# debbiemarkslab/EVcouplings

Hardware: AMD Instinct MI355X
Metric: plmc L-BFGS iterations/sec (PLM fit, synthetic MSA) (higher is better)
Workload: dtype f32 (forward: f16 hi/lo split couplings on the 2:4 sparse MFMA, f32 accumulation -- in the last iterations of a fit 39-bit fixed-point couplings as five int8 digit planes, exact; backward: 24-bit fixed-point residuals as three int8 digit planes on the int8 MFMA (32-bit / four there), exact int32 acc; 1 GPU; headline: synthetic MSA L=300 q=21 N=50000, theta=0.8, lambda_h=0.01, lambda_J=59.8; parallelism=single GPU

## Files before the change

evcouplings_amd/csrc/plm_kernels.hip:

```cpp
#include "../../include/plm_hip.h"
#include "plm_internal.h"
#include <math.h>
#include <stdlib.h>
#include <string.h>
#include <mutex>
#include <utility>

typedef _Float16 half8 __attribute__((ext_vector_type(8)));
typedef _Float16 half4 __attribute__((ext_vector_type(4)));
typedef _Float16 half16 __attribute__((ext_vector_type(16)));
typedef float f32x4 __attribute__((ext_vector_type(4)));
typedef int i32x4 __attribute__((ext_vector_type(4)));
typedef unsigned int u32;

#ifndef PLM_DMA_STAGGER_FWD
#define PLM_DMA_STAGGER_FWD 4
#endif
#ifndef PLM_DMA_STAGGER_BWD
#define PLM_DMA_STAGGER_BWD 0
#endif
typedef unsigned long long u64;
#ifndef PLM_ASYNC_A
#define PLM_ASYNC_A 1
#endif
// ... 890 lines not shown
    const double *cref = (const double *)((const float *)(A.Bt + (size_t)d.blk_per_shard * d.nksteps * TILE_G) +
                                          (size_t)d.blk_per_shard * 16 * Q) + ((size_t)b16l * 16 + r) * Q + a_lo;
    auto value = [&](int m, int a, int e) -> float { return (float)__builtin_fma((double)sum64[m][a][e], sc64, cref[a]); };
    if constexpr (MODE == FWD_STORE) {
        float4 *hj = (float4 *)A.out + ((size_t)tile * 8 + wave) * 2 * Q * 64 + lane;
#pragma unroll
        for (int a = 0; a < QG; a++) {
#pragma unroll
            for (int m = 0; m < 2; m++)
                store_hj(&hj[(size_t)(m * Q + a_lo + a) * 64], value(m, a, 0), value(m, a, 1), value(m, a, 2), value(m, a, 3));
        }
    } else {
        const int i = b16 * 16 + r;
#pragma unroll
        for (int m = 0; m < 2; m++) {
#pragma unroll
            for (int reg = 0; reg < 4; reg++) {
                const int s = s_wave + 16 * m + 4 * g + reg;
                if (i < d.L && s < d.N) {
                    float *o = A.out + ((size_t)s * d.L + i) * d.Qc + a_lo;
#pragma unroll
                    for (int a = 0; a < QG; a++)
                        if (a_lo + a < d.Qc) o[a] = value(m, a, reg);
                }
            }
        }
    }
}

template <auto KERNEL> static hipError_t plm_allow_lds(size_t lds) {
    static std::once_flag once[PLM_MAX_DEVICES];
    static hipError_t result[PLM_MAX_DEVICES];
    const int dev = plm_current_device();
    std::call_once(once[dev], [&] {
        result[dev] = lds > 65536 ? hipFuncSetAttribute((const void *)KERNEL, hipFuncAttributeMaxDynamicSharedMemorySize, (int)lds)
                                  : hipSuccess;
    });
    return result[dev];
}

#ifndef PLM_FWDW_INC
#define PLM_FWDW_INC "plm_fwd_asm.inc"
#endif
#include PLM_FWDW_INC
template <int IDX> __device__ __forceinline__ f32x4 fwdw_acc_read() {
    f32x4 v;
    asm volatile("v_accvgpr_read_b32 %0, a[%4]\n\tv_accvgpr_read_b32 %1, a[%5]\n\t"
                 "v_accvgpr_read_b32 %2, a[%6]\n\tv_accvgpr_read_b32 %3, a[%7]"
                 : "=v"(v[0]), "=v"(v[1]), "=v"(v[2]), "=v"(v[3])
                 : "n"(IDX), "n"(IDX + 1), "n"(IDX + 2), "n"(IDX + 3));
    return v;
}
template <int M, int A>
__device__ __forceinline__ void fwdw_store(float4 *hj, const float *chi, const float *clo, float sc32) {
    const f32x4 v = fwdw_acc_read<(M * PLM_FWDW_QG + A) * 4>();
    const float h = chi[A], l = clo[A];
    store_hj(&hj[(size_t)((M & 1) * 21 + A) * 64 + (size_t)(M >> 1) * 2 * 21 * 64],
             __builtin_fmaf(v[0], sc32, l) + h, __builtin_fmaf(v[1], sc32, l) + h,
             __builtin_fmaf(v[2], sc32, l) + h, __builtin_fmaf(v[3], sc32, l) + h);
}
template <int M, int... A>
__device__ __forceinline__ void fwdw_store_row(float4 *hj, const float *chi, const float *clo, float sc32, std::integer_sequence<int, A...>) {
    (fwdw_store<M, A>(hj, chi, clo, sc32), ...);
}
template <int... M>
__device__ __forceinline__ void fwdw_store_all(float4 *hj, const float *chi, const float *clo, float sc32, std::integer_sequence<int, M...>) {
    (fwdw_store_row<M>(hj, chi, clo, sc32, std::make_integer_sequence<int, PLM_FWDW_QG>{}), ...);
}

__global__ __launch_bounds__(256) void k_fwd_w(PlmDims d, FwdArgs A) {
    extern __shared__ __attribute__((aligned(16))) char smem[];
    constexpr int Q = 21, QG = PLM_FWDW_QG, NSG = Q / QG, NM = PLM_FWDW_NM, SLOT = PLM_FWDW_SLOT;
    constexpr int TILE_G = 2 * Q * 1024, NG = PLM_FWD_NG(Q), SPU = 2 * NG;
    static_assert(NG == 5 && 2 * 2 * QG * 1024 == SLOT, "plm_fwd_asm.inc is generated for 21 states in groups of 7");
    const int tid = threadIdx.x, lane = tid & 63;
    const int wv = __builtin_amdgcn_readfirstlane(tid >> 6);
    const int npair = (d.nstiles + 1) >> 1;
    const int nwork = npair * (d.b16_hi - d.b16_lo) * NSG, per_xcd = (nwork + 7) >> 3;
    const int wk = (int)(blockIdx.x & 7) * per_xcd + (int)(blockIdx.x >> 3);
    if ((int)(blockIdx.x >> 3) >= per_xcd || wk >= nwork) return;
    const int spair = wk % npair, sg = (wk / npair) % NSG, b16l = wk / (npair * NSG);
    const int a_lo = sg * QG;
    const int r = lane & 15, g = lane >> 4;
    const int stile = 2 * spair + (wv >> 1);
    const bool tile_ok = stile < d.nstiles;
    const int s_wave = tile_ok ? stile * PLM_SEQ_TILE + (wv & 1) * 128 : 0;
    const int nsteps = d.nu * SPU;
    const char *bt = A.Bt + (size_t)b16l * nsteps * 2 * TILE_G + (size_t)a_lo * 1024 + wv * 1024;
    const u32 arow = (u32)(s_wave + r) * (u32)d.Lp32 + 8 * g, rstride = 16 * (u32)d.Lp32;

    const u32 l16 = (u32)lane * 16;
    u32 vo[PLM_FWDW_NVMEM];
#pragma unroll
    for (int k = 0; k < PLM_FWDW_NVMEM; k++) {
        const int p = wv + 4 * k, run = p / QG, f = p - run * QG;
        vo[k] = l16 + (u32)((run >> 1) * TILE_G + (run & 1) * Q * 1024 + f * 1024) - (u32)wv * 1024;
    }
    const u32 lw = lds_addr(smem + lane * 16);
    const u32 lw_base = __builtin_amdgcn_readfirstlane(lw - l16);
    const u32 m0t0 = lw_base + wv * 1024;
    const u32 cnt = lw_base + 4 * SLOT;
    if (tid == 0) *(u32 *)(smem + 4 * SLOT) = 0;
    const u32 one = 1, sel = 0x0c0c0200u;
    u32 st, sp;
    asm volatile(PLM_FWDW_ZERO_ASM ::: PLM_FWDW_CLOBBERS);
    for (int i = 0; i < 3; i++) {
        const int stepc = min(i, nsteps - 1);
        asm volatile(PLM_FWDW_ISSUE_ASM
                     :
                     : [tsrc] "s"(bt + (size_t)stepc * 2 * TILE_G), [vo0] "v"(vo[0]), [vo1] "v"(vo[1]), [vo2] "v"(vo[2]),
                       [vo3] "v"(vo[3]), [vo4] "v"(vo[4]), [vo5] "v"(vo[5]), [vo6] "v"(vo[6]), [m0t] "s"(m0t0 + i * SLOT)
                     : "m0", "scc", "memory");
    }
    asm volatile(PLM_FWDW_LOADS_ASM : : [arow] "v"(arow), [rstride] "s"(rstride), [xsrc] "s"(A.msa_rm) : PLM_FWDW_CLOBBERS);
    asm volatile(PLM_FWDW_UPREP_ASM
                 :
                 : [arow] "v"(arow), [rstride] "s"(rstride), [xsrc] "s"(A.msa_rm + 32 * min(1, d.nu - 1)), [sel] "s"(sel)
                 : PLM_FWDW_CLOBBERS);
    vm_wait<0>();
    __syncthreads();
    asm volatile(PLM_FWDW_PRIME_ASM : : [kg] "s"(0), [lbn] "v"(lw) : PLM_FWDW_CLOBBERS);

    int sc = 0;
    u32 tgt = 0;
    const char *tsrc = bt + (size_t)min(3, nsteps - 1) * 2 * TILE_G;
    int step = 0;
#define FWDW_SLICE(WHICH, KG)                                                                                          \
    {                                                                                                                  \
        const int sn = (sc + 1) & 3, snn = (sc + 3) & 3;                                                               \
        asm volatile(WHICH                                                                                             \
                     : [st] "=&s"(st), [sp] "=&s"(sp)                                                                  \
                     : [lb] "v"(lw + sc * SLOT), [lbn] "v"(lw + sn * SLOT), [kg] "s"(KG), [tsrc] "s"(tsrc),          \
                       [vo0] "v"(vo[0]), [vo1] "v"(vo[1]), [vo2] "v"(vo[2]), [vo3] "v"(vo[3]), [vo4] "v"(vo[4]),       \
                       [vo5] "v"(vo[5]), [vo6] "v"(vo[6]), [m0t] "s"(m0t0 + snn * SLOT), [cnt] "v"(cnt),               \
                       [one] "v"(one), [tgt] "s"(tgt)                                                                  \
                     : PLM_FWDW_CLOBBERS);                                                                             \
        sc = sn;                                                                                                       \
        tgt += 4;                                                                                                      \
        tsrc += (step + 4 < nsteps) ? (size_t)2 * TILE_G : 0;               \
        ++step;                                                                                                        \
    }
    for (int u = 0; u < d.nu; ++u) {
#pragma unroll 1
        for (int k = 0; k < NG; ++k) {
            FWDW_SLICE(PLM_FWDW_EVEN_ASM, k)
            if (k == NG - 1)
                asm volatile(PLM_FWDW_UPREP_ASM
                             :
                             : [arow] "v"(arow), [rstride] "s"(rstride),
                               [xsrc] "s"(A.msa_rm + 32 * min(u + 2, d.nu - 1)), [sel] "s"(sel)
                             : PLM_FWDW_CLOBBERS);
            FWDW_SLICE(PLM_FWDW_ODD_ASM, k + 1 < NG ? k + 1 : 0)
        }
    }
#undef FWDW_SLICE
    asm volatile("s_waitcnt vmcnt(0) lgkmcnt(0)\n\ts_nop 15\n\ts_nop 15" ::: "memory");
    if (!tile_ok) return;
    const int je = *A.jexp;
    const double sc64 = ldexp(1.0, -je);
    const double *cref = (const double *)((const float *)(A.Bt + (size_t)d.blk_per_shard * d.nksteps * TILE_G) +
                                          (size_t)d.blk_per_shard * 16 * Q) + ((size_t)b16l * 16 + r) * Q + a_lo;
    float4 *hj = (float4 *)A.out + ((size_t)(b16l * d.nstiles + stile) * 8 + (wv & 1) * 4) * 2 * Q * 64 + (size_t)a_lo * 64 + lane;
    float chi[QG], clo[QG];
#pragma unroll
    for (int a = 0; a < QG; a++) {
        const double c = cref[a];
        chi[a] = (float)c;
        clo[a] = (float)(c - (double)chi[a]);
    }
    fwdw_store_all(hj, chi, clo, (float)sc64, std::make_integer_sequence<int, NM>{});
}

int plm_fwd_groups(int q, int exact) {
    if (!exact) return q == 32 ? 2 : 1;
    return q == 32 ? 8 : q == 21 ? 3 : q == 20 ? 4 : 1;
}
template <int Q, int MODE, int NSG, bool EXACT>
static hipError_t fwd_launch(const PlmDims &d, const FwdArgs &A, hipStream_t st) {
    const int nwork = d.nstiles * (d.b16_hi - d.b16_lo) * NSG;
    const dim3 grid(8 * ((nwork + 7) / 8)), block(512);
    const size_t lds = (size_t)2 * 2 * (Q / NSG) * 1024;
    if constexpr (EXACT) {
        hipError_t e = plm_allow_lds<k_fwd_x<Q, MODE, NSG>>(lds);
        if (e != hipSuccess) return e;
        hipLaunchKernelGGL((k_fwd_x<Q, MODE, NSG>), grid, block, lds, st, d, A);
    } else {
        hipError_t e = plm_allow_lds<k_fwd<Q, MODE, NSG>>(lds);
        if (e != hipSuccess) return e;
        hipLaunchKernelGGL((k_fwd<Q, MODE, NSG>), grid, block, lds, st, d, A);
    }
    return hipGetLastError();
}
static hipError_t fwdw_launch(const PlmDims &d, const FwdArgs &A, hipStream_t st) {
    const int nwork = ((d.nstiles + 1) / 2) * (d.b16_hi - d.b16_lo) * (21 / PLM_FWDW_QG);
    const size_t lds = (size_t)4 * PLM_FWDW_SLOT + 16;
    hipError_t e = plm_allow_lds<k_fwd_w>(lds);
    if (e != hipSuccess) return e;
    hipLaunchKernelGGL(k_fwd_w, dim3(8 * ((nwork + 7) / 8)), dim3(256), lds, st, d, A);
    return hipGetLastError();
}
static hipError_t launch_forward_mode(const PlmDims &d, const FwdArgs &A, int mode, int exact, hipStream_t st) {
    if (d.b16_hi <= d.b16_lo) return hipSuccess;
#define FWD_CASE(QQ, NP, NX)       \
    case QQ:                                                                                           \
        if (mode == FWD_ENERGY) return fwd_launch<QQ, FWD_ENERGY, NP, false>(d, A, st);                \
        if (mode == FWD_POTENTIALS && exact) return fwd_launch<QQ, FWD_POTENTIALS, NX, true>(d, A, st); \
        if (mode == FWD_POTENTIALS) return fwd_launch<QQ, FWD_POTENTIALS, NP, false>(d, A, st);        \
        if (exact) return fwd_launch<QQ, FWD_STORE, NX, true>(d, A, st);                               \
        if (QQ == 21 && d.fwd_w) return fwdw_launch(d, A, st);                                         \
        return fwd_launch<QQ, FWD_STORE, NP, false>(d, A, st);
    switch (d.Q) {
        FWD_CASE(32, 2, 8)
        FWD_CASE(21, 1, 3)
        FWD_CASE(20, 1, 4)
        FWD_CASE(5, 1, 1)
        FWD_CASE(4, 1, 1)
    default:
        return hipErrorInvalidValue;
    }
#undef FWD_CASE
}
hipError_t plm_launch_forward_energy(const PlmDims &d, const int8_t *msa_rm, const void *Bt, const float *x,
                                     const int32_t *jexp, int potentials, int exact, float *out, hipStream_t st) {
    const FwdArgs A{msa_rm, (const char *)Bt, x, jexp, out};
    return launch_forward_mode(d, A, potentials ? FWD_POTENTIALS : FWD_ENERGY, potentials ? exact : 0, st);
}
hipError_t plm_launch_forward_store(const PlmDims &d, const int8_t *msa_rm, const void *Bt, const int32_t *jexp,
                                    float *hj, int exact, hipStream_t st) {
    const FwdArgs A{msa_rm, (const char *)Bt, nullptr, jexp, hj};
    return launch_forward_mode(d, A, FWD_STORE, exact, st);
}
size_t plm_hj_bytes(const PlmDims &d) { return (size_t)d.nstiles * (d.b16_hi - d.b16_lo) * 8 * 2 * d.Q * 1024; }

#define PLM_HSTATS(Q) ((Q) + (Q) * ((Q) + 1) / 2)
__host__ __device__ constexpr int plm_qc_min(int Q) { return Q == 4 ? 2 : Q == 5 ? 5 : Q == 20 ? 6 : Q == 21 ? 21 : 22; }
#ifndef PLM_HESS_SAMPLE
#define PLM_HESS_SAMPLE 32
#endif
#ifndef PLM_NEWTON_CAP
#define PLM_NEWTON_CAP 3.0
#endif
__device__ __forceinline__ float sum_over_g(float v) {
    unsigned u = __float_as_uint(v);
    auto a = __builtin_amdgcn_permlane32_swap(u, u, false, false);
    v = __uint_as_float(a[0]) + __uint_as_float(a[1]);
    u = __float_as_uint(v);
    auto b = __builtin_amdgcn_permlane16_swap(u, u, false, false);
    return __uint_as_float(b[0]) + __uint_as_float(b[1]);
}
__device__ __forceinline__ float log_unbiased(float z) {
    const float l2 = __builtin_amdgcn_logf(z);
    return __builtin_fmaf(l2, -1.904654323148236e-9f, l2 * 0.693147182464599609375f);
}
__device__ __forceinline__ float sel_eq(int x, int a, float if_ne, float if_eq) {
    float out;
    asm("v_cmp_eq_u32 vcc, %1, %2\n\tv_cndmask_b32 %0, %3, %4, vcc" : "=v"(out) : "s"(a), "v"(x), "v"(if_ne), "v"(if_eq) : "vcc");
    return out;
}
__device__ __forceinline__ void sel_eq2(int x, int a, float ne0, float eq0, float ne1, float eq1, float &o0, float &o1) {
    asm("v_cmp_eq_u32 vcc, %2, %3\n\tv_cndmask_b32 %0, %4, %5, vcc\n\tv_cndmask_b32 %1, %6, %7, vcc"
        : "=&v"(o0), "=&v"(o1) : "s"(a), "v"(x), "v"(ne0), "v"(eq0), "v"(ne1), "v"(eq1) : "vcc");
}
__global__ void k_sum_partials(const double *__restrict__ p, int n, double *out);
struct HpassArgs {
    const float4 *hj;
    const int8_t *msa_rm;
    const float *w;
    const double *h;
    int hstride;
    char *Rt;
    double *fx_part;
    float *hpart;
    double *gpart;
    float rscale;
    double *dpart;
    const int *state;
    int cond;
    int sel;
};
__device__ __forceinline__ bool vp_runs(const int *state, int cond) {
    if (!state || cond == PLM_VP_ALWAYS) return true;
    const PlmVpState *S = (const PlmVpState *)state;
    if (cond == PLM_VP_FINAL) return S->final_skip == 0;
    if (S->done) return false;
    return cond == PLM_VP_PASS_RT ? S->want_rt != 0 : S->want_rt == 0;
}
#define PLM_HESS_PARTS(Q) (((Q) == 20 || (Q) == 21) ? 3 : 1)
template <int Q> __host__ __device__ constexpr int hess_entry0(int a) { return a * Q - a * (a - 1) / 2; }
template <int Q> __host__ __device__ constexpr int hess_row_begin(int part) {
    if (part <= 0) return 0;
    if (part >= PLM_HESS_PARTS(Q)) return Q;
    int a = 0;
    while (a < Q && hess_entry0<Q>(a) * PLM_HESS_PARTS(Q) < part * (Q * (Q + 1) / 2)) a++;
    return a;
}
template <int Q> __host__ __device__ constexpr int hess_part_entries() {
    int m = 0;
    for (int p = 0; p < PLM_HESS_PARTS(Q); p++) {
        const int n = hess_entry0<Q>(hess_row_begin<Q>(p + 1)) - hess_entry0<Q>(hess_row_begin<Q>(p));
        m = n > m ? n : m;
    }
    return m;
}
template <int Q, bool WRITE_RT, int STATS, bool XACT>
__global__ __launch_bounds__(512) void k_hpass(PlmDims d, HpassArgs A) {
    extern __shared__ __attribute__((aligned(16))) char smem[];
    constexpr int NH = (STATS == 2) ? Q * (Q + 1) / 2 : 0;
    constexpr int NSP = (STATS == 2) ? PLM_HESS_PARTS(Q) : 1;
    constexpr int NHP = (STATS == 2) ? hess_part_entries<Q>() : 0;
    if (!vp_runs(A.state, A.cond)) return;
    if (A.state) A.h += (size_t)((const PlmVpState *)A.state)->cur * A.hstride;
    const int tid = threadIdx.x, lane = tid & 63;
    const int wave = __builtin_amdgcn_readfirstlane(tid >> 6);
    const int ns1 = (d.nstiles + PLM_HESS_SAMPLE - 1) / PLM_HESS_SAMPLE;
    const int sel = A.sel;
    const int part = (int)blockIdx.x % NSP, bid = (int)blockIdx.x / NSP;
    int row_lo = 0, row_hi = Q;
    if constexpr (NSP > 1) {
        row_lo = part == 0 ? 0 : (part == 1 ? hess_row_begin<Q>(1) : hess_row_begin<Q>(2));
        row_hi = part == 0 ? hess_row_begin<Q>(1) : (part == 1 ? hess_row_begin<Q>(2) : Q);
    }
    const int ent_lo = row_lo * Q - row_lo * (row_lo - 1) / 2, ent_hi = row_hi * Q - row_hi * (row_hi - 1) / 2;
    const int nst = sel == 0 ? d.nstiles : (sel == 1 ? ns1 : d.nstiles - ns1);
    const int kt = bid % nst, b16l = bid / nst;
    if (A.state && A.cond == PLM_VP_PASS && b16l < PLM_VP_MAXBLK && ((const PlmVpState *)A.state)->quiet[b16l]) return;
    const int stile = sel == 0 ? kt : (sel == 1 ? kt * PLM_HESS_SAMPLE : kt + kt / (PLM_HESS_SAMPLE - 1) + 1);
    constexpr int HW = Q > 21 ? 2 : 8;
    constexpr bool sampled = STATS == 2, DIAG = STATS == 3 || (STATS == 2 && Q > 21);
    const int blk = b16l * d.nstiles + stile;
    const int b16 = d.b16_lo + b16l;
    const int r = lane & 15, g = lane >> 4;
    const int s_wave = stile * PLM_SEQ_TILE + wave * 32;
    const int gap = d.gap_mode;
    const int i = b16 * 16 + r;
    const bool site_ok = i < d.L;
    float hv[XACT ? 1 : Q], hl[XACT ? 1 : Q];
    double hd[XACT ? Q : 1];
    auto load_fields = [&](bool opaque) {
        u32 hoff = (u32)(site_ok ? i - d.h_site0 : 0) * Q;
        if (opaque) asm volatile("" : "+v"(hoff));
#pragma unroll
        for (int a = 0; a < Q; a++) {
            const double h64 = site_ok ? A.h[hoff + a] : 0.0;
            if constexpr (XACT) {
                hd[a] = h64;
            } else {
                hv[a] = (float)h64;
                hl[a] = (float)(h64 - (double)hv[a]);
            }
        }
    };
    constexpr bool LDSF = !WRITE_RT && !XACT && (STATS != 2 || Q > 21);
    constexpr size_t STAT_BYTES = (size_t)16 * (8 * Q * sizeof(double) * (DIAG ? 2 : 1) + HW * NHP * sizeof(float));
    float2 *lf = (float2 *)(smem + STAT_BYTES);
    constexpr bool FAST = !WRITE_RT && !XACT && (STATS == 1 || STATS == 3);
    if constexpr (LDSF) {
        for (int k = tid; k < 16 * Q; k += 512) {
            const int ii = b16 * 16 + k / Q;
            const double h64 = ii < d.L ? A.h[(size_t)(ii - d.h_site0) * Q + k % Q] : 0.0;
            const float hi = (float)h64;
            lf[k] = make_float2(hi, (float)(h64 - (double)hi));
        }
        __syncthreads();
    } else if constexpr (!WRITE_RT) load_fields(false);
    float fxl = 0.f;
    double *lg = (double *)smem + ((size_t)wave * 16 + r) * Q;
    double *ld = lg + (size_t)8 * 16 * Q;
    float *lh0 = (float *)((double *)smem + (size_t)8 * 16 * Q * (DIAG ? 2 : 1));
    float *ls = lh0 + ((size_t)wave * 16 + r) * NHP;
    if (STATS) {
        for (int k = lane; k < 16 * Q; k += 64) ((double *)smem)[(size_t)wave * 16 * Q + k] = 0.0;
        if constexpr (sampled)
            if (wave < HW)
                for (int k = lane; k < 16 * NHP; k += 64) lh0[(size_t)wave * 16 * NHP + k] = 0.f;
        if constexpr (DIAG)
            for (int k = lane; k < 16 * Q; k += 64) ((double *)smem)[(size_t)(8 + wave) * 16 * Q + k] = 0.0;
    }
    const char *hj_u = (const char *)(A.hj + ((size_t)blk * 8 + wave) * 2 * Q * 64);
    const u32 lane16 = (u32)lane * 16;
    int m_end = 2;
    asm volatile("" : "+s"(m_end));
#pragma nounroll
    for (int m = 0; m < m_end; m++) {
        if constexpr (WRITE_RT) load_fields(true);
        f32x4 acc[Q];
#pragma unroll
        for (int a = 0; a < Q; a++) {
            const float4 v = *(const float4 *)(hj_u + (size_t)(m * Q + a) * 1024 + lane16);
            acc[a] = (f32x4){v.x, v.y, v.z, v.w};
        }
        float wk[4];
        float izk[4];
        int xk[4];
#pragma unroll
        for (int reg = 0; reg < 4; reg++) {
            const int s = s_wave + 16 * m + 4 * g + reg;
            const int xi = A.msa_rm[(size_t)s * d.Lp32 + i];
            const bool skip = gap && xi == 0;
            const float ws = (skip || !site_ok) ? 0.f : A.w[s];
            float mx = -INFINITY, Z = 0.f, hx = 0.f, zo = 0.f;
            if constexpr (!XACT) {
                u32 foff = (u32)r * Q;
                if constexpr (LDSF) asm volatile("" : "+v"(foff));
#pragma unroll
                for (int a = 0; a < Q; a++) {
                    float fh, fl;
                    if constexpr (LDSF) {
                        const float2 f = lf[foff + a];
                        fh = f.x;
                        fl = f.y;
                    } else {
                        fh = hv[a];
                        fl = hl[a];
                    }
                    const float H = ((gap && a == 0) || (a >= plm_qc_min(Q) && a >= d.Qc)) ? -INFINITY : (acc[a][reg] + fl) + fh;
                    acc[a][reg] = H;
                    mx = fmaxf(mx, H);
                }
                if constexpr (FAST) {
                    const float mxl = -mx * 1.44269502f;
#pragma unroll
                    for (int a = 0; a < Q; a++) {
                        const float ev = __builtin_amdgcn_exp2f(__builtin_fmaf(acc[a][reg], 1.44269502f, mxl));
                        const float evo = sel_eq(xi, a, ev, 0.f);
                        acc[a][reg] = evo;
                        Z += ev;
                        zo += evo;
                    }
                } else {
#pragma unroll
                    for (int a = 0; a < Q; a++) {
                        const float H = acc[a][reg] - mx;
                        const float ev = __expf(H);
                        float evo;
                        sel_eq2(xi, a, hx, H, ev, 0.f, hx, evo);
                        acc[a][reg] = ev;
                        Z += ev;
                        zo += evo;
                    }
                }
            } else {
#pragma unroll
                for (int a = 0; a < Q; a++) {
                    const float H = ((gap && a == 0) || a >= d.Qc) ? -INFINITY : acc[a][reg] + (float)hd[a];
                    mx = fmaxf(mx, H);
                }
                const double mxd = (double)mx;
#pragma unroll
                for (int a = 0; a < Q; a++) {
                    const double xs = ((double)acc[a][reg] + hd[a]) - mxd;
                    const double y = xs * 1.4426950408889634;
                    const float yh = (float)y, yl = (float)(y - (double)yh);
                    const float rr = __builtin_amdgcn_exp2f(yh);
                    const float ev = ((gap && a == 0) || a >= d.Qc) ? 0.f : __builtin_fmaf(rr, yl * 0.693147182464599609375f, rr);
                    float evo;
                    sel_eq2(xi, a, hx, (float)xs, ev, 0.f, hx, evo);
                    acc[a][reg] = ev;
                    Z += ev;
                    zo += evo;
                }
            }
            const float invZ = 1.f / Z;
            if (WRITE_RT && ws > 0.f) fxl -= ws * (hx - log_unbiased(Z));
            const float mpo = -(zo * invZ);
            if constexpr (FAST) {
                if (ws != 0.f) {
                    unsafeAtomicAdd(&lg[xi], (double)(ws * mpo));
                    if constexpr (STATS == 3) {
                        const float px = 1.f + mpo;
                        unsafeAtomicAdd(&ld[xi], (double)(ws * px * px));
                    }
                }
                wk[reg] = ws * invZ;
                izk[reg] = invZ;
                xk[reg] = xi;
            } else {
#pragma unroll
            for (int a = 0; a < Q; a++) acc[a][reg] = sel_eq(xi, a, acc[a][reg] * invZ, mpo);
            wk[reg] = ws;
            xk[reg] = xi;
            }
            asm volatile("" : "+v"(xk[reg]));
            if constexpr (XACT) __builtin_amdgcn_sched_barrier(0);
        }
        if constexpr (STATS != 0) {
            int idx = 0;
#pragma unroll
            for (int a = 0; a < Q; a++) {
                float t[4], ga = 0.f;
#pragma unroll
                for (int k = 0; k < 4; k++) {
                    t[k] = wk[k] * acc[a][k];
                    ga += t[k];
                }
#ifndef PLM_EXP_NOGRAD
                if (NSP == 1 || part == 0) unsafeAtomicAdd(&lg[a], (double)ga);
#else
                fxl += ga;
#endif
                if constexpr (DIAG) {
                    float da = 0.f;
                    if constexpr (FAST) {
#pragma unroll
                        for (int k = 0; k < 4; k++) da = fmaf(t[k] * acc[a][k], izk[k], da);
                    } else {
#pragma unroll
                    for (int k = 0; k < 4; k++) {
                        const bool obs = xk[k] == a;
                        da = fmaf(t[k] + (obs ? wk[k] : 0.f), acc[a][k] + (obs ? 1.f : 0.f), da);
                    }
                    }
#ifndef PLM_EXP_NOGRAD
                    unsafeAtomicAdd(&ld[a], (double)da);
#else
                    fxl += da;
#endif
                }
#ifndef PLM_EXP_NOHESS
                if (STATS == 2 && wave < HW && a >= row_lo && a < row_hi) {
                    idx = a * Q - a * (a - 1) / 2 - ent_lo;
#pragma unroll
                    for (int k = 0; k < 4; k++) t[k] += (xk[k] == a) ? wk[k] : 0.f;
#pragma unroll
                    for (int b = a; b < Q; b++) {
                        float v = 0.f;
#pragma unroll
                        for (int k = 0; k < 4; k++) v = fmaf(t[k], acc[b][k] + ((xk[k] == b) ? 1.f : 0.f), v);
#ifndef PLM_EXP_NOSWAP
                        v = sum_over_g(v);
#endif
#ifndef PLM_EXP_NOLDS
                        if (g == 0) __builtin_amdgcn_ds_faddf(LDS_FPTR(&ls[idx]), v, 0, 0, false);
#else
                        fxl += v;
#endif
                        ++idx;
                    }
                }
#endif
            }
        }
        if constexpr (WRITE_RT) {
            __builtin_amdgcn_sched_barrier(0);
            const int s64 = stile * 4 + (wave >> 1);
            const int Gq = 2 * (wave & 1) + m;
            char *rt_u = A.Rt + rt_slot(d, 0, s64, b16l * Q, 0);
            const size_t rt_plane = (size_t)d.nst128 * d.nnfl * 2048;
            const u32 slot16 = (u32)(Gq * 16 + r) * 16;
#pragma unroll
            for (int reg = 0; reg < 4; reg++) {
                wk[reg] *= A.rscale;
                asm volatile("" : "+v"(xk[reg]));
            }
            const bool four = d.nplanes == 4;
            auto planes_of_state = [&](int a, u32 (&pl)[PLM_BWD_MAXPLANES]) {
                u32 x[4];
#pragma unroll
                for (int reg = 0; reg < 4; reg++)
                    x[reg] = digits_of(wk[reg] * acc[a][reg], four);
                planes_of4(x[0], x[1], x[2], x[3], pl);
            };
#pragma unroll
            for (int q4 = 0; q4 + 4 <= Q; q4 += 4) {
                u32 pl[4][PLM_BWD_MAXPLANES];
#pragma unroll
                for (int k = 0; k < 4; k++) planes_of_state(q4 + k, pl[k]);
                const u32 off = (u32)(q4 + g) * 2048 + slot16;
#pragma unroll
                for (int p = 0; p < PLM_BWD_MAXPLANES; p++) {
                    if (p >= d.nplanes) break;
                    auto s02 = __builtin_amdgcn_permlane32_swap(pl[0][p], pl[2][p], false, false);
                    auto s13 = __builtin_amdgcn_permlane32_swap(pl[1][p], pl[3][p], false, false);
                    auto t0 = __builtin_amdgcn_permlane16_swap(s02[0], s13[0], false, false);
                    auto t1 = __builtin_amdgcn_permlane16_swap(s02[1], s13[1], false, false);
                    *(uint4 *)(rt_u + p * rt_plane + off) = make_uint4(t0[0], t0[1], t1[0], t1[1]);
                }
                __builtin_amdgcn_sched_barrier(0);
            }
#pragma unroll
            for (int a = Q - Q % 4; a < Q; a++) {
                u32 pl[PLM_BWD_MAXPLANES];
                planes_of_state(a, pl);
#pragma unroll
                for (int p = 0; p < PLM_BWD_MAXPLANES; p++)
                    if (p < d.nplanes) *(u32 *)(rt_u + p * rt_plane + (u32)a * 2048 + slot16 + 4 * g) = pl[p];
            }
        }
    }
    __syncthreads();
    if constexpr (STATS != 0) {
        if (NSP == 1 || part == 0) {
            double *gout = A.gpart + (size_t)blk * 16 * Q;
            for (int k = tid; k < 16 * Q; k += 512) {
                double v = 0;
#pragma unroll
                for (int wv = 0; wv < 8; wv++) v += ((const double *)smem)[(size_t)wv * 16 * Q + k];
                gout[k] = v;
            }
        }
        if constexpr (DIAG) {
            double *dout = A.dpart + (size_t)blk * 16 * Q;
            for (int k = tid; k < 16 * Q; k += 512) {
                double v = 0;
#pragma unroll
                for (int wv = 0; wv < 8; wv++) v += ((const double *)smem)[(size_t)(8 + wv) * 16 * Q + k];
                dout[k] = v;
            }
        }
        if constexpr (sampled) {
            float *out = A.hpart + (size_t)blk * 16 * NH;
            const int ne = ent_hi - ent_lo;
            for (int k = tid; k < 16 * ne; k += 512) {
                const int site = k / ne, e = k - site * ne;
                float v = 0.f;
#pragma unroll
                for (int wv = 0; wv < HW; wv++) v += lh0[((size_t)wv * 16 + site) * NHP + e];
                out[site * NH + ent_lo + e] = v;
            }
        }
    }
    if constexpr (WRITE_RT) {
        __syncthreads();
        const double tot = block_reduce_sum((double)fxl, (double *)smem);
        if (tid == 0) A.fx_part[blk] = tot;
    }
}
hipError_t plm_launch_hpass(const PlmDims &d, const float *hj, const int8_t *msa_rm, const float *w,
                            const double *h64, int write_rt, int stats, int exact, void *Rt, double *fx_part, float *hpart,
                            double *gpart, double *dpart, const int *state, int cond, hipStream_t st) {
    if (d.b16_hi <= d.b16_lo) return hipSuccess;
    const int nb = d.b16_hi - d.b16_lo, ns1 = (d.nstiles + PLM_HESS_SAMPLE - 1) / PLM_HESS_SAMPLE;
    const dim3 block(512);
    HpassArgs A{(const float4 *)hj, msa_rm, w, h64, (int)plm_h64_stride(d), (char *)Rt, fx_part,
                hpart, gpart, d.rscale, dpart, state, cond, 0};
#define HP_LAUNCH(QQ, WW, SS)                                                                          \
    {                                                                                                  \
        const dim3 grid((A.sel == 0 ? d.nstiles : (A.sel == 1 ? ns1 * ((SS) == 2 ? PLM_HESS_PARTS(QQ) : 1) : d.nstiles - ns1)) * nb); \
        const size_t lds = (size_t)16 * (8 * (QQ) * sizeof(double) * (((SS) == 3 || ((SS) == 2 && (QQ) > 21)) ? 2 : 1) + \
                                         ((SS) == 2 ? ((QQ) > 21 ? 2 : 8) * hess_part_entries<QQ>() : 0) * sizeof(float)) + \
                           (size_t)16 * (QQ) * sizeof(float2);           \
        {                                                                                              \
            hipError_t e = exact ? plm_allow_lds<k_hpass<QQ, WW, SS, true>>(lds) : plm_allow_lds<k_hpass<QQ, WW, SS, false>>(lds); \
            if (e != hipSuccess) return e;                                                             \
        }                                                                                              \
        if (exact) hipLaunchKernelGGL((k_hpass<QQ, WW, SS, true>), grid, block, lds, st, d, A);        \
        else hipLaunchKernelGGL((k_hpass<QQ, WW, SS, false>), grid, block, lds, st, d, A);             \
    }
#define HP_CASE(QQ)                                                                                    \
    case QQ:                                                                                           \
        if (write_rt && stats == 2) return hipErrorInvalidValue;    \
        else if (write_rt && stats == 0) HP_LAUNCH(QQ, true, 0)                                        \
        else if (write_rt) HP_LAUNCH(QQ, true, 1)                                                      \
        else if (stats == 2) {                                                                         \
            if (!dpart) return hipErrorInvalidValue;                                                   \
                         \
            A.sel = 1;                                                                                 \
            HP_LAUNCH(QQ, false, 2)                                                                    \
            A.sel = 2;                                                                                 \
            if (d.nstiles > ns1) HP_LAUNCH(QQ, false, 3)                                               \
        } else HP_LAUNCH(QQ, false, 1)                                                                 \
        break;
    switch (d.Q) {
        HP_CASE(32)
        HP_CASE(21)
        HP_CASE(20)
        HP_CASE(5)
        HP_CASE(4)
    default:
        return hipErrorInvalidValue;
    }
#undef HP_CASE
#undef HP_LAUNCH
    return hipGetLastError();
}
size_t plm_hpart_bytes(const PlmDims &d) {
    return (size_t)d.nstiles * (d.b16_hi - d.b16_lo) * 16 * (d.Q * (d.Q + 1) / 2) * sizeof(float);
}
size_t plm_h64_stride(const PlmDims &d) {
    const size_t nsites = (size_t)std::max(std::max(1, (d.b16_hi - d.b16_lo) * 16), std::min(d.L, d.own_hi * 16) - d.h_site0);
    return nsites * d.Q;
}
size_t plm_gpart_bytes(const PlmDims &d) { return (size_t)d.nstiles * (d.b16_hi - d.b16_lo) * 16 * d.Q * sizeof(double); }

template <int Q>
__global__ __launch_bounds__(256) void k_site_counts(PlmDims d, const int8_t *__restrict__ msa_cm, const float *__restrict__ w,
                                                    double *__restrict__ cnt) {
    __shared__ double red[4];
    const int il = blockIdx.x, i = d.h_site0 + il;
    double acc[Q];
#pragma unroll
    for (int a = 0; a < Q; a++) acc[a] = 0.0;
    if (i < d.L)
        for (int s = threadIdx.x; s < d.N; s += 256) {
            const int x = msa_cm[(size_t)i * d.Np + s];
            const double ws = (d.gap_mode && x == 0) ? 0.0 : (double)w[s];
#pragma unroll
            for (int a = 0; a < Q; a++) acc[a] += (x == a) ? ws : 0.0;
        }
#pragma unroll
    for (int a = 0; a < Q; a++) {
        const double t = block_reduce_sum(acc[a], red);
        if (threadIdx.x == 0) cnt[(size_t)il * Q + a] = t;
        __syncthreads();
    }
}
hipError_t plm_launch_site_counts(const PlmDims &d, const int8_t *msa_cm, const float *w, double *cnt, hipStream_t st) {
    const int nsites = (d.b16_hi - d.b16_lo) * 16;
    if (nsites <= 0) return hipSuccess;
    switch (d.Q) {
    case 32: hipLaunchKernelGGL(k_site_counts<32>, dim3(nsites), dim3(256), 0, st, d, msa_cm, w, cnt); break;
    case 21: hipLaunchKernelGGL(k_site_counts<21>, dim3(nsites), dim3(256), 0, st, d, msa_cm, w, cnt); break;
    case 20: hipLaunchKernelGGL(k_site_counts<20>, dim3(nsites), dim3(256), 0, st, d, msa_cm, w, cnt); break;
    case 5: hipLaunchKernelGGL(k_site_counts<5>, dim3(nsites), dim3(256), 0, st, d, msa_cm, w, cnt); break;
    case 4: hipLaunchKernelGGL(k_site_counts<4>, dim3(nsites), dim3(256), 0, st, d, msa_cm, w, cnt); break;
    default: return hipErrorInvalidValue;
    }
    return hipGetLastError();
}

template <int Q>
__global__ __launch_bounds__(64) void k_hsolve(PlmDims d, const float *__restrict__ hpart,
                                              const double *__restrict__ gpart, int full,
                                              float *__restrict__ x, double *__restrict__ h64,
                                              double lambda_h, int update,
                                              double *__restrict__ hinv, double *__restrict__ g2_site,
                                              double tol_site2, const int *__restrict__ state, int chain, int hstride,
                                              const double *__restrict__ cnt, const double *__restrict__ dpart) {
    constexpr int NVF = PLM_HSTATS(Q);
    const PlmVpState *S = (const PlmVpState *)state;
    int cur = 0;
    if (S) {
        if (chain && S->done) return;
        if (full == 2) full = S->want_rt ? 0 : 1;
        cur = S->cur;
    } else if (full == 2) full = 1;
    __shared__ double st[NVF];
    __shared__ double Hm[Q][2 * Q + 1];
    __shared__ double Hi[Q][Q + 1];
    __shared__ double gr[Q], Dv[Q], mv[Q], Md[Q];
    const int il = blockIdx.x, t = threadIdx.x;
    const int i = d.h_site0 + il;
    if (i >= min(d.L, d.own_hi * 16)) {
        if (t == 0) g2_site[il] = 0.0;
        return;
    }
    const double *hc = h64 + (size_t)cur * hstride + (size_t)il * Q;
    double *hn = h64 + (size_t)((S && chain) ? (cur ^ 1) : cur) * hstride + (size_t)il * Q;
    const int b16l = il >> 4, r = il & 15;
    const bool quiet = S && chain && b16l < PLM_VP_MAXBLK && S->quiet[b16l];
    if (quiet) {
        if (update && t < Q) hn[t] = hc[t];
        if (!S->want_rt) return;
        update = 0;
        full = 0;
    }
    constexpr int NH = Q * (Q + 1) / 2;
    {
        double part[Q];
#pragma unroll
        for (int k = 0; k < Q; k++) part[k] = 0;
        for (int tt = t; tt < d.nstiles; tt += 128) {
            const bool two = tt + 64 < d.nstiles;
            const double *src0 = gpart + (((size_t)b16l * d.nstiles + tt) * 16 + r) * Q;
            const double *src1 = gpart + (((size_t)b16l * d.nstiles + (two ? tt + 64 : tt)) * 16 + r) * Q;
            double v0[Q], v1[Q];
#pragma unroll
            for (int k = 0; k < Q; k++) { v0[k] = src0[k]; v1[k] = src1[k]; }
#pragma unroll
            for (int k = 0; k < Q; k++) { part[k] += v0[k]; if (two) part[k] += v1[k]; }
        }
#pragma unroll
        for (int k = 0; k < Q; k++) {
            double v = part[k];
            for (int o = 32; o > 0; o >>= 1) v += __shfl_xor(v, o, 64);
            if (t == 0) st[k] = v;
        }
    }
    if (full) {
        const int nsamp = (d.nstiles + PLM_HESS_SAMPLE - 1) / PLM_HESS_SAMPLE;
        for (int k = t; k < NH; k += 64) {
            double v = 0;
            for (int j0 = 0; j0 < nsamp; j0 += 8) {
                float u[8];
#pragma unroll
                for (int j = 0; j < 8; j++) {
                    const int tt = min(j0 + j, nsamp - 1) * PLM_HESS_SAMPLE;
                    u[j] = hpart[(((size_t)b16l * d.nstiles + tt) * 16 + r) * NH + k];
                }
#pragma unroll
                for (int j = 0; j < 8; j++)
                    if (j0 + j < nsamp) v += (double)u[j];
            }
            st[Q + k] = v * ((double)d.nstiles / nsamp) * (Q > 21 ? 4.0 : 1.0);
        }
        if (dpart) {
            double part[Q];
#pragma unroll
            for (int k = 0; k < Q; k++) part[k] = 0;
            for (int tt0 = t; tt0 < d.nstiles; tt0 += 128) {
                const bool two = tt0 + 64 < d.nstiles;
                double v[2][Q];
#pragma unroll
                for (int h = 0; h < 2; h++) {
                    const int tt = (h && two) ? tt0 + 64 : tt0;
                    const size_t blk = ((size_t)b16l * d.nstiles + tt) * 16 + r;
                    if (Q <= 21 && (tt % PLM_HESS_SAMPLE) == 0) {
#pragma unroll
                        for (int k = 0; k < Q; k++) v[h][k] = (double)hpart[blk * NH + (k * Q - k * (k - 1) / 2)];
                    } else {
#pragma unroll
                        for (int k = 0; k < Q; k++) v[h][k] = dpart[blk * Q + k];
                    }
                }
#pragma unroll
                for (int k = 0; k < Q; k++) { part[k] += v[0][k]; if (two) part[k] += v[1][k]; }
            }
#pragma unroll
            for (int k = 0; k < Q; k++) {
                double v = part[k];
                for (int o = 32; o > 0; o >>= 1) v += __shfl_xor(v, o, 64);
                if (t == 0) Md[k] = v;
            }
        }
    }
    __syncthreads();
    const int a0 = d.gap_mode;
    if (t < Q) gr[t] = (t < a0) ? 0.0 : st[t] + 2.0 * lambda_h * hc[t];
    __syncthreads();
    double *inv = hinv + (size_t)il * Q * Q;
    if (full) {
        for (int k = t; k < Q * Q; k += 64) {
            const int a = k / Q, b = k % Q, lo = min(a, b), hi = max(a, b);
            Hm[a][b] = -st[Q + lo * Q - lo * (lo - 1) / 2 + (hi - lo)];
            Hm[a][Q + b] = (a == b) ? 1.0 : 0.0;
        }
        __syncthreads();
        const bool xdiag = cnt && dpart;
        if (t < Q) {
            mv[t] = cnt ? fmax(0.0, st[t] + cnt[(size_t)il * Q + t]) : 0.0;
            if (xdiag) {
                mv[t] = fmax(0.0, mv[t] - Md[t]);
                Hm[t][t] = 0.0;
            }
            Dv[t] = 1.0;
        }
        __syncthreads();
        if (cnt) {
            for (int sweep = 0; sweep < 3; sweep++) {
                double nd = 0.0;
                if (t < Q) {
                    double rs = 0;
                    for (int b = 0; b < Q; b++) rs -= Hm[t][b] * Dv[b];
                    rs *= Dv[t];
                    nd = rs > 0.0 ? Dv[t] * sqrt(mv[t] / rs) : 0.0;
                }
                __syncthreads();
                if (t < Q) Dv[t] = nd;
                __syncthreads();
            }
            for (int k = t; k < Q * Q; k += 64) Hm[k / Q][k % Q] *= Dv[k / Q] * Dv[k % Q];
            __syncthreads();
        }
        if (t < Q) {
            double rowsum = 0;
            for (int b = 0; b < Q; b++) rowsum -= Hm[t][b];
            Hm[t][2 * Q] = rowsum;
        }
        __syncthreads();
        if (t < Q) Hm[t][t] += Hm[t][2 * Q] + 2.0 * lambda_h + 1e-12 * (1.0 + Hm[t][2 * Q]);
        __syncthreads();
        {
            double col[Q];
            const int tc = min(t, 2 * Q - 1);
#pragma unroll
            for (int a = 0; a < Q; a++) col[a] = Hm[a][tc];
#pragma unroll
            for (int p = 0; p < Q; p++) {
                const double piv = 1.0 / lane_bcast(col[p], p);
                col[p] *= piv;
#pragma unroll
                for (int a = 0; a < Q; a++) {
                    if (a == p) continue;
                    const double f = lane_bcast(col[a], p);
                    col[a] -= f * col[p];
                }
            }
            if (t >= Q && t < 2 * Q) {
#pragma unroll
                for (int a = 0; a < Q; a++) Hm[a][t] = col[a];
            }
            __syncthreads();
        }
    }
    double g2 = 0;
    for (int a = 0; a < Q; a++) g2 += gr[a] * gr[a];
    if (t == 0) g2_site[il] = g2;
    const bool move = update && g2 > tol_site2;
    if (!move && !full) {
        if (S && chain && update && t < Q) hn[t] = hc[t];
        return;
    }
    for (int k = t; k < Q * Q; k += 64) Hi[k / Q][k % Q] = full ? Hm[k / Q][Q + k % Q] : inv[k];
    __syncthreads();
    const bool dirty = full != 0;
    if (dirty) for (int k = t; k < Q * Q; k += 64) inv[k] = Hi[k / Q][k % Q];
    if (!move) {
        if (S && chain && update && t < Q) hn[t] = hc[t];
        return;
    }
    double dh = 0;
    if (t < Q) {
        for (int b = 0; b < Q; b++) dh += Hi[t][b] * gr[b];
        if (t < a0) dh = 0;
    }
    double mxs = fabs(dh);
    for (int o = 32; o > 0; o >>= 1) mxs = fmax(mxs, __shfl_xor(mxs, o, 64));
    const double cap = (mxs > PLM_NEWTON_CAP) ? PLM_NEWTON_CAP / mxs : 1.0;
    if (t < Q) {
        const bool bad = mxs != mxs;
        const double hnew = bad ? hc[t] : hc[t] - cap * dh;
        hn[t] = hnew;
        if (!(S && chain)) x[(size_t)il * Q + t] = (float)hnew;
    }
}
__global__ __launch_bounds__(256) void k_fields_to_x(const double *__restrict__ h64, const int *__restrict__ state, int hstride,
                                                    float *__restrict__ x, int n) {
    const int k = blockIdx.x * 256 + threadIdx.x;
    const int cur = state ? ((const PlmVpState *)state)->cur : 0;
    if (k < n) x[k] = (float)h64[(size_t)cur * hstride + k];
}
hipError_t plm_launch_fields_to_x(const PlmDims &d, const double *h64, const int *state, float *x, hipStream_t st) {
    const int n = (std::min(d.L, d.own_hi * 16) - d.h_site0) * d.Q;
    if (n <= 0) return hipSuccess;
    hipLaunchKernelGGL(k_fields_to_x, dim3((n + 255) / 256), dim3(256), 0, st, h64, state, (int)plm_h64_stride(d), x, n);
    return hipGetLastError();
}
__global__ __launch_bounds__(256) void k_h64_init(const float *__restrict__ x, double *__restrict__ h64, int n) {
    const int k = blockIdx.x * 256 + threadIdx.x;
    if (k < n) h64[k] = (double)x[k];
}
hipError_t plm_launch_h64_init(const PlmDims &d, const float *x, double *h64, hipStream_t st) {
    const int n = (std::min(d.L, d.own_hi * 16) - d.h_site0) * d.Q;
    if (n <= 0) return hipSuccess;
    hipLaunchKernelGGL(k_h64_init, dim3((n + 255) / 256), dim3(256), 0, st, x, h64, n);
    return hipGetLastError();
}
__global__ __launch_bounds__(256) void k_vp_check(const double *__restrict__ g2_site, int n, double *g2_out,
                                                 double tol_site2, double tol2, double floor2, int *state) {
    __shared__ double red[4];
    __shared__ int bad[4];
    PlmVpState *S = (PlmVpState *)state;
    if (S && S->done) {
        if (threadIdx.x == 0) {
            g2_out[1] = (double)S->passes;
            g2_out[2] = 1.0;
        }
        return;
    }
// ... 1323 lines not shown
```

Measured before the change: 113.1 iterations/s.

## Fuse sampled Hessian and diagonal hpass launches into one grid, restructure Hessian accumulation

Merges the two stats==2 hpass launches (sampled Hessian tiles and the remaining diagonal-only tiles) into a single kernel grid that dispatches on block index. The sampled Hessian path is rewritten to unroll rows at compile time in descending order, batch eight entries per cross-lane permlane32/16 reduction, and use fields staged in LDS. Launch bounds are raised to four waves per SIMD for this path, and global stores use precomputed per-plane address-space-1 base pointers. The aim is to remove one launch plus its tail, and to cut reduction and address overhead. In exchange there is a larger LDS footprint and more register pressure from the higher occupancy bound.

Result: no change. 113.1 iterations/s (median of 4 runs) (-0.1%).

```diff
diff --git a/evcouplings_amd/csrc/plm_kernels.hip b/evcouplings_amd/csrc/plm_kernels.hip
--- a/evcouplings_amd/csrc/plm_kernels.hip
+++ b/evcouplings_amd/csrc/plm_kernels.hip
@@ -1216,8 +1216,11 @@
     }
     return m;
 }
+template <int... I, class F> __device__ __forceinline__ void rows_downwards(std::integer_sequence<int, I...>, F &&f) {
+    (f(std::integral_constant<int, (int)sizeof...(I) - 1 - I>{}), ...);
+}
 template <int Q, bool WRITE_RT, int STATS, bool XACT>
-__global__ __launch_bounds__(512) void k_hpass(PlmDims d, HpassArgs A) {
+__device__ __forceinline__ void hpass_body(const PlmDims &d, HpassArgs A, const int bidx) {
     extern __shared__ __attribute__((aligned(16))) char smem[];
     constexpr int NH = (STATS == 2) ? Q * (Q + 1) / 2 : 0;
     constexpr int NSP = (STATS == 2) ? PLM_HESS_PARTS(Q) : 1;
@@ -1228,7 +1231,7 @@
     const int wave = __builtin_amdgcn_readfirstlane(tid >> 6);
     const int ns1 = (d.nstiles + PLM_HESS_SAMPLE - 1) / PLM_HESS_SAMPLE;
     const int sel = A.sel;
-    const int part = (int)blockIdx.x % NSP, bid = (int)blockIdx.x / NSP;
+    const int part = bidx % NSP, bid = bidx / NSP;
     int row_lo = 0, row_hi = Q;
     if constexpr (NSP > 1) {
         row_lo = part == 0 ? 0 : (part == 1 ? hess_row_begin<Q>(1) : hess_row_begin<Q>(2));
@@ -1251,11 +1254,12 @@
     float hv[XACT ? 1 : Q], hl[XACT ? 1 : Q];
     double hd[XACT ? Q : 1];
     auto load_fields = [&](bool opaque) {
-        u32 hoff = (u32)(site_ok ? i - d.h_site0 : 0) * Q;
+        u32 hoff = (u32)(site_ok ? i - d.h_site0 : 0) * (Q * (u32)sizeof(double));
         if (opaque) asm volatile("" : "+v"(hoff));
+        const double *hp = (const double *)((const char *)A.h + hoff);
 #pragma unroll
         for (int a = 0; a < Q; a++) {
-            const double h64 = site_ok ? A.h[hoff + a] : 0.0;
+            const double h64 = site_ok ? hp[a] : 0.0;
             if constexpr (XACT) {
                 hd[a] = h64;
             } else {
@@ -1264,7 +1268,7 @@
             }
         }
     };
-    constexpr bool LDSF = !WRITE_RT && !XACT && (STATS != 2 || Q > 21);
+    constexpr bool LDSF = !WRITE_RT && !XACT;
     constexpr size_t STAT_BYTES = (size_t)16 * (8 * Q * sizeof(double) * (DIAG ? 2 : 1) + HW * NHP * sizeof(float));
     float2 *lf = (float2 *)(smem + STAT_BYTES);
     constexpr bool FAST = !WRITE_RT && !XACT && (STATS == 1 || STATS == 3);
@@ -1397,8 +1401,7 @@
             asm volatile("" : "+v"(xk[reg]));
             if constexpr (XACT) __builtin_amdgcn_sched_barrier(0);
         }
-        if constexpr (STATS != 0) {
-            int idx = 0;
+        if constexpr (STATS != 0 && !sampled) {
 #pragma unroll
             for (int a = 0; a < Q; a++) {
                 float t[4], ga = 0.f;
@@ -1430,29 +1433,69 @@
                     fxl += da;
 #endif
                 }
-#ifndef PLM_EXP_NOHESS
-                if (STATS == 2 && wave < HW && a >= row_lo && a < row_hi) {
-                    idx = a * Q - a * (a - 1) / 2 - ent_lo;
-#pragma unroll
-                    for (int k = 0; k < 4; k++) t[k] += (xk[k] == a) ? wk[k] : 0.f;
-#pragma unroll
-                    for (int b = a; b < Q; b++) {
-                        float v = 0.f;
-#pragma unroll
-                        for (int k = 0; k < 4; k++) v = fmaf(t[k], acc[b][k] + ((xk[k] == b) ? 1.f : 0.f), v);
-#ifndef PLM_EXP_NOSWAP
-                        v = sum_over_g(v);
-#endif
-#ifndef PLM_EXP_NOLDS
-                        if (g == 0) __builtin_amdgcn_ds_faddf(LDS_FPTR(&ls[idx]), v, 0, 0, false);
-#else
-                        fxl += v;
-#endif
-                        ++idx;
+            }
+        }
+        if constexpr (sampled) {
+            const bool grads = NSP == 1 || part == 0;
+            float *const lsb = lh0 + ((int)(((u32)wave * 16 + r) * NHP) - ent_lo);
+            constexpr int EB = 8;
+            rows_downwards(std::make_integer_sequence<int, Q>{}, [&](auto row) __attribute__((always_inline)) {
+                constexpr int a = decltype(row)::value;
+                if (a < row_lo && !grads && !DIAG) return;
+                float t[4], ga = 0.f;
+#pragma unroll
+                for (int k = 0; k < 4; k++) {
+                    t[k] = wk[k] * acc[a][k];
+                    ga += t[k];
+                }
+                if (grads) unsafeAtomicAdd(&lg[a], (double)ga);
+#pragma unroll
+                for (int k = 0; k < 4; k++) {
+                    const bool obs = xk[k] == a;
+                    t[k] += obs ? wk[k] : 0.f;
+                    acc[a][k] += obs ? 1.f : 0.f;
+                }
+                if constexpr (DIAG) {
+                    float da = 0.f;
+#pragma unroll
+                    for (int k = 0; k < 4; k++) da = fmaf(t[k], acc[a][k], da);
+                    unsafeAtomicAdd(&ld[a], (double)da);
+                }
+                if (wave < HW && a >= row_lo && a < row_hi) {
+#pragma unroll
+                    for (int b0 = a; b0 < Q; b0 += EB) {
+                        float v[EB];
+#pragma unroll
+                        for (int j = 0; j < EB; j++) {
+                            v[j] = 0.f;
+                            if (b0 + j < Q) {
+#pragma unroll
+                                for (int k = 0; k < 4; k++) v[j] = fmaf(t[k], acc[b0 + j][k], v[j]);
+                            }
+                        }
+#pragma unroll
+                        for (int j = 0; j < EB; j++)
+                            if (b0 + j < Q) {
+                                const unsigned u = __float_as_uint(v[j]);
+                                auto sw = __builtin_amdgcn_permlane32_swap(u, u, false, false);
+                                v[j] = __uint_as_float(sw[0]) + __uint_as_float(sw[1]);
+                            }
+#pragma unroll
+                        for (int j = 0; j < EB; j++)
+                            if (b0 + j < Q) {
+                                const unsigned u = __float_as_uint(v[j]);
+                                auto sw = __builtin_amdgcn_permlane16_swap(u, u, false, false);
+                                v[j] = __uint_as_float(sw[0]) + __uint_as_float(sw[1]);
+                            }
+                        if (g == 0) {
+#pragma unroll
+                            for (int j = 0; j < EB; j++)
+                                if (b0 + j < Q)
+                                    __builtin_amdgcn_ds_faddf(LDS_FPTR(&lsb[hess_entry0<Q>(a) + (b0 - a) + j]), v[j], 0, 0, false);
+                        }
                     }
                 }
-#endif
-            }
+            });
         }
         if constexpr (WRITE_RT) {
             __builtin_amdgcn_sched_barrier(0);
@@ -1461,6 +1504,17 @@
             char *rt_u = A.Rt + rt_slot(d, 0, s64, b16l * Q, 0);
             const size_t rt_plane = (size_t)d.nst128 * d.nnfl * 2048;
             const u32 slot16 = (u32)(Gq * 16 + r) * 16;
+            typedef __attribute__((address_space(1))) char gchar;
+            typedef u32 u32x4 __attribute__((ext_vector_type(4)));
+            typedef __attribute__((address_space(1))) u32x4 guint4;
+            typedef __attribute__((address_space(1))) u32 gu32;
+            gchar *rt_p[PLM_BWD_MAXPLANES];
+#pragma unroll
+            for (int p = 0; p < PLM_BWD_MAXPLANES; p++) {
+                char *bp = rt_u + p * rt_plane;
+                asm volatile("" : "+s"(bp));
+                rt_p[p] = (gchar *)bp;
+            }
 #pragma unroll
             for (int reg = 0; reg < 4; reg++) {
                 wk[reg] *= A.rscale;
@@ -1487,7 +1541,9 @@
                     auto s13 = __builtin_amdgcn_permlane32_swap(pl[1][p], pl[3][p], false, false);
                     auto t0 = __builtin_amdgcn_permlane16_swap(s02[0], s13[0], false, false);
                     auto t1 = __builtin_amdgcn_permlane16_swap(s02[1], s13[1], false, false);
-                    *(uint4 *)(rt_u + p * rt_plane + off) = make_uint4(t0[0], t0[1], t1[0], t1[1]);
+                    u32 o = off;
+                    asm volatile("" : "+v"(o));
+                    *(guint4 *)(rt_p[p] + o) = (u32x4){t0[0], t0[1], t1[0], t1[1]};
                 }
                 __builtin_amdgcn_sched_barrier(0);
             }
@@ -1497,7 +1553,7 @@
                 planes_of_state(a, pl);
 #pragma unroll
                 for (int p = 0; p < PLM_BWD_MAXPLANES; p++)
-                    if (p < d.nplanes) *(u32 *)(rt_u + p * rt_plane + (u32)a * 2048 + slot16 + 4 * g) = pl[p];
+                    if (p < d.nplanes) *(gu32 *)(rt_p[p] + ((u32)a * 2048 + slot16 + 4 * (u32)g)) = pl[p];
             }
         }
     }
@@ -1537,6 +1593,43 @@
         __syncthreads();
         const double tot = block_reduce_sum((double)fxl, (double *)smem);
         if (tid == 0) A.fx_part[blk] = tot;
+    }
+}
+template <int Q, bool WRITE_RT, int STATS, bool XACT> constexpr int hpass_waves() { return (STATS == 2 && !WRITE_RT && !XACT && Q <= 21) ? 4 : 2; }
+template <int Q, bool WRITE_RT, int STATS, bool XACT>
+__global__ __launch_bounds__(512, (hpass_waves<Q, WRITE_RT, STATS, XACT>())) void k_hpass(PlmDims d, HpassArgs A) {
+    hpass_body<Q, WRITE_RT, STATS, XACT>(d, A, (int)blockIdx.x);
+}
+template <int Q>
+__global__ __launch_bounds__(512, 4) void k_hpass_hess(PlmDims d, HpassArgs A, int n1) {
+    if ((int)blockIdx.x < n1) {
+        A.sel = 1;
+        hpass_body<Q, false, 2, false>(d, A, (int)blockIdx.x);
+    } else {
+        A.sel = 2;
+        hpass_body<Q, false, 3, false>(d, A, (int)blockIdx.x - n1);
+    }
+}
+static bool hpass_one_grid() {
+    static const bool on = [] {
+        const char *e = getenv("PLM_HPASS_ONE_GRID");
+        return !(e && e[0] == '0');
+    }();
+    return on;
+}
+template <int Q> static hipError_t launch_hpass_hess(const PlmDims &d, const HpassArgs &A, int ns1, int nb, hipStream_t st) {
+    if constexpr (Q <= 21) {
+        const int n1 = ns1 * PLM_HESS_PARTS(Q) * nb;
+        const dim3 grid(n1 + (d.nstiles - ns1) * nb), block(512);
+        const size_t lds = (size_t)16 * std::max(8 * Q * sizeof(double) + 8 * hess_part_entries<Q>() * sizeof(float),
+                                                 8 * Q * sizeof(double) * 2) +
+                           (size_t)16 * Q * sizeof(float2);
+        const hipError_t e = plm_allow_lds<k_hpass_hess<Q>>(lds);
+        if (e != hipSuccess) return e;
+        hipLaunchKernelGGL((k_hpass_hess<Q>), grid, block, lds, st, d, A, n1);
+        return hipSuccess;
+    } else {
+        return hipErrorInvalidValue;
     }
 }
 hipError_t plm_launch_hpass(const PlmDims &d, const float *hj, const int8_t *msa_rm, const float *w,
@@ -1567,7 +1660,12 @@
         else if (write_rt) HP_LAUNCH(QQ, true, 1)                                                      \
         else if (stats == 2) {                                                                         \
             if (!dpart) return hipErrorInvalidValue;                                                   \
-                         \
+                                                                             \
+            if ((QQ) <= 21 && !exact && d.nstiles > ns1 && hpass_one_grid()) {                         \
+                const hipError_t e = launch_hpass_hess<QQ>(d, A, ns1, nb, st);                         \
+                if (e != hipSuccess) return e;                                                         \
+                break;                                                                                 \
+            }                                                                                          \
             A.sel = 1;                                                                                 \
             HP_LAUNCH(QQ, false, 2)                                                                    \
             A.sel = 2;                                                                                 \
```
